# ShannonAI/GNN-LM

Hardware: AMD Instinct MI355X
Metric: eval tokens/sec on WikiText-103 (k=1024, GNN+KNN); test ppl match (higher is better)
Workload: dtype f32

## Files before the change

### gnn-lm_amd/csrc/ivfpq8_scan.hip

```cpp
#include "kernels.h"
#include "ivfpq8_layout.h"

namespace gnnlm {
namespace {

typedef int v4i __attribute__((ext_vector_type(4)));
typedef int v8i __attribute__((ext_vector_type(8)));
typedef unsigned u32x2 __attribute__((ext_vector_type(2)));
typedef unsigned v4u __attribute__((ext_vector_type(4)));

#define GNNLM_PERM(hi_, lo_, sel_) __builtin_amdgcn_perm((hi_), (lo_), (sel_))
#ifndef GNNLM_IVF8_NW
#define GNNLM_IVF8_NW 16
#endif
constexpr int NW = GNNLM_IVF8_NW, NTH = 64 * NW;
#ifndef GNNLM_IVF8_PF
#define GNNLM_IVF8_PF 3
#endif
#ifndef GNNLM_IVF8_PF_SUMS
#define GNNLM_IVF8_PF_SUMS 3
#endif
template <bool SUMS>
__global__ __launch_bounds__(NTH) void ivfpq_scan8_kernel(gnnlm_ivfpq_scan8_t p) {
    extern __shared__ __attribute__((aligned(16))) unsigned char smem[];
// ... 235 lines not shown
        for (int q = 0; q < 4; ++q) lookups4(C[0], q, X[q]);
#define GNNLM_IVF8_STEP(t) if constexpr (PF > (t)) { step(C[((t) + 1) % PF], C[(t)], u); u += NW * TS; }
        while (u < nt) {
            GNNLM_IVF8_STEP(0) GNNLM_IVF8_STEP(1) GNNLM_IVF8_STEP(2) GNNLM_IVF8_STEP(3)
            GNNLM_IVF8_STEP(4) GNNLM_IVF8_STEP(5) GNNLM_IVF8_STEP(6) GNNLM_IVF8_STEP(7)
        }
#undef GNNLM_IVF8_STEP
        static_assert(PF >= 3 && PF <= 8, "GNNLM_IVF8_PF");
    }
    if (SUMS) {
        __syncthreads();
#pragma unroll
        for (int u = 0; u < QG; ++u) {
            const int64_t ob = p.grp_out[(int64_t)grp * QG + u];
            if (qs[u] < 0 || ob < 0) continue;
            for (int e = tid; e < HIST_BINS; e += NTH) p.out_hist[ob + e] = hist[u * HIST_BINS + e];
        }
        advance_slow();
        continue;
    }
    count_entries(wgc);
    if (tid == 0) *next_s = next_index();
    __syncthreads();
    if (tid < QG) {
        const int tot = wgc[tid];
        wgc[tid] = (tot > 0 && qs_lane >= 0) ? atomicAdd(&p.surv_cnt[(int64_t)qs_lane * SURV_CNT_STRIDE], tot) : 0;
    }
    __syncthreads();
    gi_next = *next_s;
    write_entries(wgc);
    }
}

__global__ __launch_bounds__(1024) void ivfpq_tau_kernel(gnnlm_ivfpq_tau_t p) {
    constexpr int CB = 2 * HIST_BINS;
    __shared__ int comb[CB];
    __shared__ int part[1024];
    __shared__ int bstar_s;
    const int tid = threadIdx.x;
    const int64_t q = blockIdx.x;
    const float delta = p.qmeta[q * 4], sum_lo = p.qmeta[q * 4 + 1], amax = p.qmeta[q * 4 + 2];
    float bmin = INFINITY, bmax = -INFINITY;
    for (int d = 0; d < p.D; ++d) {
        if (p.probe_list[q * p.ld_probe + d] < 0) continue;
        const float b = p.probe_bias[q * p.ld_probe + d];
        bmin = fminf(bmin, b);
        bmax = fmaxf(bmax, b);
    }
    int c0 = 0, c1 = 0;
    for (int d = 0; d < p.D; ++d) {
        if (p.probe_list[q * p.ld_probe + d] < 0) continue;
        const float offf = (p.probe_bias[q * p.ld_probe + d] - bmin) / delta * 0.9999f - 1.f;
        const int sh = (int)fminf(fmaxf(offf, 0.f), (float)(HIST_BINS << HIST_SHIFT)) >> HIST_SHIFT;
        const uint32_t* h = p.hist + (q * p.D + d) * HIST_BINS;
        const int b0 = tid - sh, b1 = tid + 1024 - sh;
        if (b0 >= 0 && b0 < HIST_BINS) c0 += (int)h[b0];
        if (b1 >= 0 && b1 < HIST_BINS) c1 += (int)h[b1];
    }
    comb[tid] = c0;
    comb[tid + 1024] = c1;
    if (tid == 0) bstar_s = -1;
    __syncthreads();
    const int h0 = comb[2 * tid], h1 = comb[2 * tid + 1], mine = h0 + h1;
    part[tid] = mine;
    __syncthreads();
    int suf = mine;
    for (int step = 1; step < 1024; step <<= 1) {
        const int other = tid + step < 1024 ? part[tid + step] : 0;
        __syncthreads();
        suf += other;
        part[tid] = suf;
        __syncthreads();
    }
    if (suf >= p.k && suf - mine < p.k) bstar_s = (suf - mine + h1 >= p.k) ? 2 * tid + 1 : 2 * tid;
    __syncthreads();
    if (tid == 0) {
        float tau = -INFINITY;
        if (bstar_s >= 0) {
            const float eps = 66.f * 2.3841858e-7f * (64.f * amax + fmaxf(fabsf(bmin), fabsf(bmax)));
            tau = (bmin + sum_lo) + (float)(bstar_s << HIST_SHIFT) * delta * (1.f - 6.1035156e-5f) - eps;
            tau -= fabsf(tau) * 2.3841858e-7f + 1e-30f;
        }
        p.tau[q] = tau;
    }
}

}

int ivfpq_scan8(const gnnlm_ivfpq_scan8_t& d, hipStream_t stream) {
    GNNLM_REQUIRE(d.max_groups >= 0, "ivfpq_scan8: bad group count");
    if (d.max_groups == 0) return OK;
    GNNLM_REQUIRE(d.tiles && d.list_off && d.qlut && d.qmeta && d.coarse && d.grp_list && d.grp_q && d.n_groups &&
                      (d.out_hist || (d.tau && d.surv && d.surv_cnt && d.cap > 0)),
                  "ivfpq_scan8: null operand");
    GNNLM_REQUIRE(d.M == 64 && (uintptr_t)d.tiles % 16 == 0 && (uintptr_t)d.qlut % 4 == 0, "ivfpq_scan8: need M = 64, aligned images");
    GNNLM_REQUIRE(!d.out_hist || d.grp_out, "ivfpq_scan8: out_hist needs grp_out");
    GNNLM_REQUIRE(d.nlist > 0 && d.nlist <= (1 << SURV_LIST_BITS) && d.max_list >= 0 && d.max_list < (1ll << SURV_ROW_BITS),
                  "ivfpq_scan8: the survivor records hold 18 bits of list and 19 bits of row: need 0 < nlist <= 2^18 and max_list < 2^19");
    GNNLM_LDS_OPT_IN(&ivfpq_scan8_kernel<false>, scan8_lds(false));
    GNNLM_LDS_OPT_IN(&ivfpq_scan8_kernel<true>, scan8_lds(true));
    ProfScope prof(d.out_hist ? K_IVF8S : K_IVF8, stream, 0.0, 0.0);
    int dev = 0, cus = 0;
    GNNLM_HIP(hipGetDevice(&dev));
    GNNLM_HIP(hipDeviceGetAttribute(&cus, hipDeviceAttributeMultiprocessorCount, dev));
    const dim3 grid((unsigned)scan8_grid(d.max_groups, cus));
    if (d.out_hist) hipLaunchKernelGGL(ivfpq_scan8_kernel<true>, grid, dim3(NTH), scan8_lds(true), stream, d);
    else hipLaunchKernelGGL(ivfpq_scan8_kernel<false>, grid, dim3(NTH), scan8_lds(false), stream, d);
    GNNLM_LAUNCH_CHECK();
    return OK;
}

int ivfpq_tau(const gnnlm_ivfpq_tau_t& d, hipStream_t stream) {
    GNNLM_REQUIRE(d.n >= 0 && d.n < (1ll << 31) && d.D >= 1 && d.k > 0, "ivfpq_tau: bad shape");
    if (d.n == 0) return OK;
    GNNLM_REQUIRE(d.hist && d.probe_list && d.probe_bias && d.qmeta && d.tau && d.ld_probe >= d.D, "ivfpq_tau: null operand");
    ProfScope prof(K_TAU, stream, 0.0, 4.0 * (double)d.n * d.D * HIST_BINS);
    hipLaunchKernelGGL(ivfpq_tau_kernel, dim3((unsigned)d.n), dim3(1024), 0, stream, d);
    GNNLM_LAUNCH_CHECK();
    return OK;
}

}
```

### gnn-lm_amd/csrc/ivfpq_select.hip

```cpp
#include <cmath>
#include <cstdint>

#include "kernels.h"

namespace gnnlm {
namespace {

__device__ __forceinline__ uint32_t key_of(float v) {
    const uint32_t u = __float_as_uint(v);
    return (u & 0x80000000u) ? ~u : (u | 0x80000000u);
}
__device__ __forceinline__ float value_of_key(uint32_t key) { return __uint_as_float((key & 0x80000000u) ? (key & 0x7fffffffu) : ~key); }

struct ProbeParams {
    const float* scores; int64_t ld; int64_t n; int ncols;
    const float* col_bias;
    int k, largest;
    float* out_val; int64_t* out_id;
};

__device__ __forceinline__ int wave_count(bool pred) { return __popcll(__ballot(pred)); }

template <int NCH>
__global__ __launch_bounds__(256) void ivfpq_select_probes_kernel(ProbeParams p) {
// ... 87 lines not shown
    for (int r = 0; r < NR; ++r) {
        const int col = 256 * (r / 4) + 4 * lane + (r % 4);
        uint64_t m = __ballot(key[r] > T || (key[r] == T && col <= C));
        while (m) {
            const int src = __builtin_ctzll(m);
            m &= m - 1;
            const uint32_t kv = (uint32_t)__builtin_amdgcn_readlane((int)key[r], src);
            if (lane == base) { okey = kv; ocol = 256 * (r / 4) + 4 * src + (r % 4); }
            ++base;
        }
    }
    unsigned long long s = okey ? ((unsigned long long)okey << 32) | (unsigned)(4095 - ocol) : 0ull;
#pragma unroll
    for (int size = 2; size <= 64; size <<= 1) {
#pragma unroll
        for (int d = size >> 1; d > 0; d >>= 1) {
            const unsigned long long o = __shfl_xor(s, d, 64);
            const bool keep_max = ((lane & d) == 0) == ((lane & size) == 0);
            s = keep_max ? (s > o ? s : o) : (s < o ? s : o);
        }
    }
    if (lane < p.k) {
        const uint32_t kk = (uint32_t)(s >> 32);
        p.out_val[row * p.k + lane] = kk ? sign * value_of_key(kk) : (p.largest ? NEG : INFINITY);
        p.out_id[row * p.k + lane] = kk ? (int64_t)(4095 - (int)(uint32_t)s) : (int64_t)-1;
    }
}

struct FinalParams {
    const float* val; int64_t ld_val; const int64_t* ids; int64_t ld_ids;
    const int32_t* row_ncols; int64_t n; int cap, k;
    float* out_val; int64_t* out_id;
    int label_bits; int32_t val_last; int32_t* out_vals;
};

template <int EPT>
__global__ __launch_bounds__(256) void ivfpq_select_final_kernel(FinalParams p) {
    constexpr int NT = 256, NB = 2048, KP = 1024;
    __shared__ int64_t id[2][KP];
    __shared__ float val[2][KP];
    __shared__ int hist[NB];
    __shared__ int wtot[4];
    __shared__ float wext[4][2];
    __shared__ int dig_s, above_s, cnt;
    const int tid = threadIdx.x, lane = tid & 63, wave = tid >> 6;
    const int64_t row = blockIdx.x;
    const float NEG = -INFINITY;
    const float* srow = p.val + row * p.ld_val;
    const int64_t* irow = p.ids + row * p.ld_ids;
    const int ncols = p.row_ncols ? min(p.cap, p.row_ncols[row]) : p.cap;
    auto entry = [&](int c, float& v, uint32_t& key, int64_t& cid) -> bool {
        v = srow[c] + 0.f;
        cid = irow[c];
        key = key_of(v);
        return cid >= 0 && v > NEG;
    };
    auto pick = [&](int need) -> int {
        int own[8], mine = 0;
#pragma unroll
        for (int b = 0; b < 8; ++b) { own[b] = hist[8 * tid + b]; mine += own[b]; }
        int suf = mine;
#pragma unroll
        for (int d = 1; d < 64; d <<= 1) {
            const int o = __shfl_down(suf, d, 64);
            if (lane + d < 64) suf += o;
        }
        if (lane == 0) wtot[wave] = suf;
        if (tid == 0) { dig_s = -1; above_s = 0; }
        __syncthreads();
        for (int w = wave + 1; w < 4; ++w) suf += wtot[w];
        if (suf >= need && suf - mine < need) {
            int acc_ = suf - mine;
#pragma unroll
            for (int b = 7; b >= 0; --b) {
                if (acc_ + own[b] >= need) { dig_s = 8 * tid + b; above_s = acc_; break; }
                acc_ += own[b];
            }
        }
        __syncthreads();
        return dig_s;
    };
    uint32_t rkey[EPT];
    int64_t rid[EPT];
// ... 151 lines not shown
            if (p.label_bits > 0 && p.out_vals) p.out_vals[o] = (int32_t)(pid & ((1ll << p.label_bits) - 1));
        }
    }
    for (int e = m + tid; e < p.k; e += NT) {
        const int64_t o = row * p.k + e;
        p.out_val[o] = NEG;
        p.out_id[o] = -1;
        if (p.label_bits > 0 && p.out_vals) p.out_vals[o] = p.val_last;
    }
}

}

int ivfpq_select_probes(const gnnlm_ivfpq_select_probes_t& d, hipStream_t stream) {
    GNNLM_REQUIRE(d.out_val && d.out_id && d.k > 0 && d.k <= 64, "ivfpq_select_probes: need output buffers and 0 < k <= 64");
    GNNLM_REQUIRE(d.n >= 0 && d.n < (1ll << 31) && d.ncols >= 0 && d.ncols <= 4096, "ivfpq_select_probes: need 0 <= ncols <= 4096");
    if (d.n == 0) return OK;
    GNNLM_REQUIRE(d.ncols == 0 || d.scores, "ivfpq_select_probes: null scores");
    ProbeParams p{d.scores, d.ld, d.n, d.ncols, d.col_bias, d.k, d.largest, d.out_val, d.out_id};
    ProfScope prof(K_TOPK, stream, 0.0, 4.0 * (double)d.n * d.ncols + 12.0 * (double)d.n * d.k);
    const dim3 grid((unsigned)cdiv(d.n, 4)), block(256);
    if (d.ncols <= 256) hipLaunchKernelGGL(ivfpq_select_probes_kernel<1>, grid, block, 0, stream, p);
    else if (d.ncols <= 1024) hipLaunchKernelGGL(ivfpq_select_probes_kernel<4>, grid, block, 0, stream, p);
    else hipLaunchKernelGGL(ivfpq_select_probes_kernel<16>, grid, block, 0, stream, p);
    GNNLM_LAUNCH_CHECK();
    return OK;
}

int ivfpq_select_final(const gnnlm_ivfpq_select_final_t& d, hipStream_t stream) {
    GNNLM_REQUIRE(d.out_val && d.out_id && d.k > 0 && d.k <= 1024, "ivfpq_select_final: need output buffers and 0 < k <= 1024");
    GNNLM_REQUIRE(d.n >= 0 && d.n < (1ll << 31) && d.cap >= 0 && d.cap <= 16384, "ivfpq_select_final: need 0 <= cap <= 16384");
    GNNLM_REQUIRE(d.label_bits >= 0 && d.label_bits < 32, "ivfpq_select_final: need 0 <= label_bits < 32");
    if (d.n == 0) return OK;
    GNNLM_REQUIRE(d.cap == 0 || (d.cand_val && d.cand_id), "ivfpq_select_final: null candidates");
    FinalParams p{d.cand_val, d.ld_val, d.cand_id, d.ld_id, d.row_ncols, d.n, d.cap, d.k, d.out_val, d.out_id,
                  d.label_bits, d.val_last, d.out_vals};
    ProfScope prof(K_TOPK, stream, 0.0, 12.0 * (double)d.n * d.cap + 16.0 * (double)d.n * d.k);
    const dim3 grid((unsigned)d.n), block(256);
    if (d.cap <= 4096) hipLaunchKernelGGL(ivfpq_select_final_kernel<16>, grid, block, 0, stream, p);
    else hipLaunchKernelGGL(ivfpq_select_final_kernel<20>, grid, block, 0, stream, p);
    GNNLM_LAUNCH_CHECK();
    return OK;
}

}
```

### gnn-lm_amd/ivfpq.py

```python
import contextlib
import ctypes
import os
from collections import namedtuple
from typing import NamedTuple, Optional

import numpy as np
import torch

from . import _lib, ivfpq_train, ops


class _LazyStats(dict):

    def add(self, key, thunk):
        dict.setdefault(self, key, 0)
        self.__dict__.setdefault("_pending", {}).setdefault(key, []).append(thunk)

    def set(self, key, value):
        dict.__setitem__(self, key, value)

    def _resolve(self, key):
        pend = self.__dict__.get("_pending", {}).pop(key, None)
        if pend:
            dict.__setitem__(self, key, dict.__getitem__(self, key) + sum(t() for t in pend))
# ... 389 lines not shown
            _lib.call("gnnlm_ivfpq_pack_lut", _lib.ptr(blk.lut), blk.lut.stride(0), nq, self.M, _lib.ptr(lut_s), _lib.stream())
        ov = torch.empty(nq, dense * self.max_list, device=dev, dtype=torch.float32)
        self._scan(lut_s, blk, 0, dense, out=ov)
        ops.topk_merge(ov, bv, bi, largest=True, init=True)
        lst = torch.gather(pi, 1, torch.div(bi, self.max_list, rounding_mode="floor").clamp_(0, dense - 1))
        pos = self.list_off[lst.clamp(min=0)] + bi % self.max_list
        bi.copy_(torch.where(torch.isinf(bv) | (lst < 0), torch.full_like(bi, -1), self.payload[pos.clamp_(0, max(self.ntotal - 1, 0))]))
        if plan.nprobe <= dense:
            return None
        tau = torch.where(bi[:, k - 1] >= 0, bv[:, k - 1], torch.full_like(bv[:, k - 1], float("-inf"))).contiguous()
        self._scan(lut_s, blk, dense, plan.nprobe, filt=(tau, plan.cap))
        stats.add("candidates", lambda cc=blk.cc: cc.sum().double())
        if self.keep_candidates:
            self.last_candidates = (blk.cv, blk.ci, blk.cc, tau)
        ops.topk_merge(blk.cv, bv, bi, ids=blk.ci, largest=True, init=False, row_ncols=blk.cc.clamp(max=plan.cap))
        return blk.cc

    def _block_int8(self, plan, blk, out, stats):
        dev, nq, pi, cc = self.device, blk.pv.shape[0], blk.pi, blk.cc
        hist = torch.empty(nq, plan.dense, self.HIST_BINS, device=dev, dtype=torch.int32)
        self._scan8(blk.tables, blk.cs, self._groups(pi[:, :plan.dense], seg=self.HIST_BINS), hist=hist, stride=plan.S)
        tau = self._tau(plan, blk, hist)
        surv = torch.empty(nq, plan.cap, 2, device=dev, dtype=torch.int32)
        sc16 = torch.zeros(nq, self.CNT_STRIDE, device=dev, dtype=torch.int32)
        g2 = self._groups(pi)
        stats.add("groups", lambda g=g2[2]: g[0].double())
        self._scan8(blk.tables, blk.cs, g2, filt=(tau, surv, sc16))
        sc = sc16[:, 0]
        self._rescore(plan, blk, (tau, surv, sc16), stats)
        stats.add("survivors", lambda sc=sc: sc.sum().double())
        stats.add("candidates", lambda cc=cc: cc.sum().double())
        if self.keep_candidates:
            self.last_candidates = (blk.cv, blk.ci, cc, tau)
        self._select_final(plan, blk, out)
        over = sc
        if plan.ccap < plan.cap:
            over = torch.where(cc > plan.ccap, torch.full_like(sc, self.COLUMNS), over)
        if plan.S > 1:
            avail = self.list_len[pi.clamp(min=0)].masked_fill(pi < 0, 0).sum(1)
            short = cc.to(torch.int64) < avail.clamp(max=plan.k)
            stats.add("underflow", lambda short=short: short.sum().double())
            over = torch.where(short, torch.full_like(sc, self.UNDERFLOW), over)
        return over

    def _select_probes(self, plan, cs, pv, pi, col_bias=None):
        ops.ivfpq_select_probes(cs, pv, pi, col_bias, plan.select)

    def _tables_begin(self, qr):
        nq, dev = qr.shape[0], self.device
        lut = torch.empty(nq, self.M * 256, device=dev, dtype=torch.float32)
        tables = side = None
        if self.route == "int8":
            tables = (torch.empty(nq, *self.QLUT_SHAPE, dtype=torch.uint8, device=dev), torch.empty(nq, self.QMETA, dtype=torch.float32, device=dev))
            if not torch.cuda.is_current_stream_capturing():
                cur = torch.cuda.current_stream()
                side = self._side_streams.get(cur.cuda_stream)
                if side is None:
                    side = self._side_streams[cur.cuda_stream] = torch.cuda.Stream(device=dev)
                side.wait_stream(cur)
        with torch.cuda.stream(side) if side is not None else contextlib.nullcontext():
            if tables is not None and self.dsub in (4, 8, 16, 32):
                t = _lib.gnnlm_ivfpq_tables_t()
                t.qr, t.ld_qr, t.n, t.pq, t.M, t.dsub = qr.data_ptr(), qr.stride(0), nq, self.pq.data_ptr(), self.M, self.dsub
                t.lut, t.ld_lut, t.qlut, t.qmeta = lut.data_ptr(), lut.stride(0), tables[0].data_ptr(), tables[1].data_ptr()
                _lib.call_desc("gnnlm_ivfpq_tables", t)
                return lut, tables, side
            g = _lib.gnnlm_gemm_t()
# ... 48 lines not shown
        d.qlut, d.qmeta, d.coarse, d.ld_coarse = tables[0].data_ptr(), tables[1].data_ptr(), cs.data_ptr(), cs.stride(0)
        d.grp_list, d.grp_q, d.n_groups, d.max_groups = groups[0].data_ptr(), groups[1].data_ptr(), groups[2].data_ptr(), groups[3]
        ctr = torch.zeros(*self.WORK_CTR_SHAPE, device=self.device, dtype=torch.int32)
        d.work_ctr = ctr.data_ptr()
        if hist is not None:
            d.out_hist, d.grp_out = hist.data_ptr(), groups[4].data_ptr()
        else:
            tau, surv, cnt = filt
            d.tau, d.surv, d.surv_cnt, d.cap = tau.data_ptr(), surv.data_ptr(), cnt.data_ptr(), surv.shape[1]
        _lib.call_desc("gnnlm_ivfpq_scan8", d)

    def _tau(self, plan, blk, hist):
        tau = torch.empty(hist.shape[0], device=self.device, dtype=torch.float32)
        t = _lib.gnnlm_ivfpq_tau_t()
        t.hist, t.D = hist.data_ptr(), plan.dense
        t.probe_list, t.probe_bias, t.ld_probe = blk.pi.data_ptr(), blk.pv.data_ptr(), blk.pi.stride(0)
        t.qmeta, t.n, t.k, t.tau = blk.tables[1].data_ptr(), hist.shape[0], plan.rank, tau.data_ptr()
        _lib.call_desc("gnnlm_ivfpq_tau", t)
        return tau

    def _rescore(self, plan, blk, filt, stats):
        tau, surv, sc16 = filt
        r = _lib.gnnlm_ivfpq_rescore_t()
        r.codes, r.payload, r.M = self.list_codes.data_ptr(), self.payload.data_ptr(), self.M
        r.lut, r.ld_lut, r.coarse, r.ld_coarse, r.tau = blk.lut.data_ptr(), blk.lut.stride(0), blk.cs.data_ptr(), blk.cs.stride(0), tau.data_ptr()
        r.surv, r.surv_cnt, r.cap, r.n = surv.data_ptr(), sc16.data_ptr(), plan.cap, sc16.shape[0]
        r.cand_val, r.cand_id, r.cand_cnt, r.cand_cap = blk.cv.data_ptr(), blk.ci.data_ptr(), blk.cc.data_ptr(), plan.ccap
        if self.refine_tau:
            rc16 = torch.empty_like(sc16)
            r.qmeta, r.k, r.out_cnt = blk.tables[1].data_ptr(), plan.k, rc16.data_ptr()
            stats.add("rescored", lambda rc=rc16: rc[:, 0].sum().double())
        _lib.call_desc("gnnlm_ivfpq_rescore", r)

    def _select_final(self, plan, blk, out):
        cv, ci, ccap = blk.cv, blk.ci, plan.ccap
        if not (plan.k <= 1024 and (out.split or plan.select)):
            return ops.topk_merge(cv, out.val, out.idx, ids=ci, largest=True, init=True, row_ncols=blk.cc.clamp(max=ccap))
        rn = blk.cc.clamp(max=ccap)
        f = _lib.gnnlm_ivfpq_select_final_t()
        f.cand_val, f.ld_val, f.cand_id, f.ld_id = cv.data_ptr(), cv.stride(0), ci.data_ptr(), ci.stride(0)
        f.row_ncols, f.n, f.cap, f.k, f.out_val, f.out_id = rn.data_ptr(), cv.shape[0], ccap, plan.k, out.val.data_ptr(), out.idx.data_ptr()
        if out.split:
            f.label_bits, f.val_last = self.LABEL_BITS, self.val_last
            if out.labels is not None:
                f.out_vals = out.labels.data_ptr()
        _lib.call_desc("gnnlm_ivfpq_select_final", f)
```

### include/gnnlm.h

```cpp
#ifndef GNNLM_H
#define GNNLM_H

#include <stddef.h>
#include <stdint.h>

#ifdef __cplusplus
extern "C" {
#endif

#define GNNLM_ABI_VERSION 12
#define GNNLM_OK 0
#define GNNLM_E_INVALID (-22)
#define GNNLM_E_NOMEM (-12)
#define GNNLM_E_HIP (-5)

const char* gnnlm_last_error(void);
int gnnlm_abi_version(void);
const char* gnnlm_target_arch(void);
size_t gnnlm_sizeof(const char* struct_name);

typedef struct gnnlm_gemm {
    const float* A;  int64_t lda;
    const int32_t* a_rows;
    const float* W;  int64_t ldw;
// ... 279 lines not shown
    const int32_t* n_groups;  int32_t max_groups;
    uint32_t* surv;  int32_t* surv_cnt;  int32_t cap;
    uint32_t* out_hist;  const int64_t* grp_out;
    int32_t sums_stride;
    int32_t* work_ctr;
    int32_t nlist;  int64_t max_list;
} gnnlm_ivfpq_scan8_t;
int gnnlm_ivfpq_scan8(const gnnlm_ivfpq_scan8_t* desc, void* stream);
typedef struct gnnlm_ivfpq_tau {
    const uint32_t* hist;  int32_t D;
    const int64_t* probe_list;  const float* probe_bias;  int32_t ld_probe;
    const float* qmeta;
    int64_t n;  int32_t k;
    float* tau;
} gnnlm_ivfpq_tau_t;
int gnnlm_ivfpq_tau(const gnnlm_ivfpq_tau_t* desc, void* stream);
int gnnlm_ivfpq_split_payload(int64_t* idx, int64_t n, int32_t label_bits, int32_t val_last, int32_t* out_vals, void* stream);
typedef struct gnnlm_ivfpq_select_probes {
    const float* scores;  int64_t ld;
    int64_t n;  int32_t ncols;
    const float* col_bias;
    int32_t k;
    int32_t largest;
    float* out_val;  int64_t* out_id;
} gnnlm_ivfpq_select_probes_t;
int gnnlm_ivfpq_select_probes(const gnnlm_ivfpq_select_probes_t* desc, void* stream);
typedef struct gnnlm_ivfpq_select_final {
    const float* cand_val;  int64_t ld_val;
    const int64_t* cand_id;  int64_t ld_id;
    const int32_t* row_ncols;
    int64_t n;  int32_t cap;  int32_t k;
    float* out_val;  int64_t* out_id;
    int32_t label_bits;  int32_t val_last;  int32_t* out_vals;
} gnnlm_ivfpq_select_final_t;
int gnnlm_ivfpq_select_final(const gnnlm_ivfpq_select_final_t* desc, void* stream);
typedef struct gnnlm_ivfpq_rescore {
    const uint8_t* codes;  const int64_t* payload;
    int32_t M;
    const float* lut;  int64_t ld_lut;
    const float* coarse;  int64_t ld_coarse;
    const float* tau;
    const uint32_t* surv;  const int32_t* surv_cnt;  int32_t cap;
    int64_t n;
    float* cand_val;  int64_t* cand_id;  int32_t* cand_cnt;  int32_t cand_cap;
    const float* qmeta;  int32_t k;  int32_t* out_cnt;
} gnnlm_ivfpq_rescore_t;
int gnnlm_ivfpq_rescore(const gnnlm_ivfpq_rescore_t* desc, void* stream);
typedef struct gnnlm_ivfpq_encode {
    const float* x;  int64_t ldx;  int64_t n;
    const int64_t* assign;
    const float* coarse;  int32_t nlist;
    const float* pq;  const float* norm2;
    int32_t M;  int32_t dsub;  int32_t d;
    uint8_t* codes;  int64_t ld_codes;
    int64_t* list_cnt;  int32_t* n_bad;
} gnnlm_ivfpq_encode_t;
int gnnlm_ivfpq_encode_rows(const gnnlm_ivfpq_encode_t* desc, void* stream);
typedef struct gnnlm_ivfpq_list_merge {
    const int64_t* list_off_old;  int32_t nlist;  int64_t N0;
    const int64_t* ids_old;  const uint8_t* codes_old;  int32_t M;
    int64_t n;  const int64_t* dest;  const int64_t* ids_new;  const uint8_t* codes_new;  int64_t ld_new;
    const int64_t* new_off;
    int64_t* ids;  uint8_t* codes;
    int32_t* n_bad;
} gnnlm_ivfpq_list_merge_t;
int gnnlm_ivfpq_list_merge(const gnnlm_ivfpq_list_merge_t* desc, void* stream);
typedef struct gnnlm_ivfpq_coarse {
// ... 302 lines not shown
```

### gnn-lm_amd/csrc/ivfpq8_layout.h

```cpp
#pragma once
#include <stddef.h>
#include <stdint.h>

#if defined(__HIPCC__)
#include <hip/hip_runtime.h>
#define GNNLM_HD __host__ __device__
#else
#define GNNLM_HD
#endif

namespace gnnlm {

constexpr int QG = 8;
constexpr int TQ = 32;
constexpr int QLUT_BYTES = 64 * 256;
constexpr int TAB_BYTES = 2 * 256 * 32 * QG;
#ifndef GNNLM_IVF8_WAVE_CAP
#define GNNLM_IVF8_WAVE_CAP 240
#endif
constexpr int WAVE_CAP = GNNLM_IVF8_WAVE_CAP;
constexpr int SCAN_CTL = 768;
constexpr int SCAN_LDS = TAB_BYTES + SCAN_CTL + 16 * WAVE_CAP * 8;
constexpr int HIST_BINS = 1024, HIST_SHIFT = 4;
constexpr int SUMS_LDS = TAB_BYTES + QG * HIST_BINS * 4;
constexpr int SURV_CNT_STRIDE = 16;
static_assert(TAB_BYTES == QG * QLUT_BYTES, "a group's LDS tables are its queries' byte tables, interleaved");
static_assert(SCAN_LDS <= 160 * 1024 && SUMS_LDS <= 160 * 1024, "the scan's tables + staging regions / histograms exceed a CU's LDS");

constexpr int SURV_ROW_BITS = 19, SURV_LIST_BITS = 18, SURV_EXCESS_MAX = 254, SURV_SUM_BIG = 16383;
static_assert(SURV_SUM_BIG == (1 << (32 - SURV_LIST_BITS)) - 1 && SURV_SUM_BIG > 16320, "list and sum share the record's second word");
struct SurvRec { uint32_t row, word; };
GNNLM_HD constexpr SurvRec surv_pack(uint32_t row, uint32_t list, uint32_t sum) { return SurvRec{row, list | sum << SURV_LIST_BITS}; }
GNNLM_HD constexpr uint32_t surv_list(uint32_t word) { return word & ((1u << SURV_LIST_BITS) - 1u); }
GNNLM_HD constexpr uint32_t surv_sum(uint32_t word) { return word >> SURV_LIST_BITS; }

constexpr int64_t ivf8_cdiv(int64_t a, int64_t b) { return (a + b - 1) / b; }
constexpr int64_t groups_cap(int64_t n, int64_t P, int64_t nlist) { return n * P / QG + nlist + 1; }
constexpr int64_t groups_fill(int64_t G, int64_t nlist) { return G * QG > 2 * (nlist + 1) ? G * QG : 2 * (nlist + 1); }
constexpr int64_t scan8_grid(int64_t max_groups, int64_t cus) {
    const int64_t by_groups = 8 * ivf8_cdiv(max_groups, 8), by_cus = 8 * ivf8_cdiv(cus > 8 ? cus : 8, 8);
    return by_groups < by_cus ? by_groups : by_cus;
}
constexpr size_t scan8_lds(bool sums) { return sums ? SUMS_LDS : SCAN_LDS; }
constexpr size_t rescore_lds(int M, int threads) { return (size_t)M * 256 * 4 + (size_t)threads * M; }
constexpr int64_t tables_grid(int64_t n) { return ivf8_cdiv(n, TQ); }

#if defined(__HIPCC__)
__device__ __forceinline__ int filter_threshold(const float* __restrict__ qmeta, int64_t q, float bias, float tau) {
    const float delta = qmeta[q * 4], sum_lo = qmeta[q * 4 + 1], amax = qmeta[q * 4 + 2];
    const float eps = 66.f * 2.3841858e-7f * (64.f * amax + fabsf(bias) + (fabsf(tau) < INFINITY ? fabsf(tau) : 0.f));
    const float thr = ((tau - bias) - sum_lo - eps) / delta - 64.f;
    return !(thr == thr) || thr <= -1.0e9f ? -(1 << 30) : (thr >= 1.0e9f ? 0x7fffffff : (int)floorf(thr) - 128 * 64);
}
#endif

}
```

### gnn-lm_amd/csrc/ivfpq8_rescore.hip

```cpp
#include "kernels.h"
#include "ivfpq8_layout.h"

namespace gnnlm {
namespace {

typedef unsigned v4u __attribute__((ext_vector_type(4)));
#ifndef GNNLM_REFINE_NT
#define GNNLM_REFINE_NT 1024
#endif
template <int EPT>
__device__ __forceinline__ void refine_wg(const gnnlm_ivfpq_rescore_t& p, const int64_t q, int* hist, int& n_left, float& tau_left) {
    constexpr int NT = GNNLM_REFINE_NT, NB = 2048, NWV = NT / 64;
    __shared__ int wtot[NWV];
    __shared__ int dig_s, base_s;
    const int tid = threadIdx.x, lane = tid & 63, wave = tid >> 6;
    const int n = min(p.surv_cnt[q * SURV_CNT_STRIDE], p.cap);
    uint2* surv = reinterpret_cast<uint2*>(const_cast<uint32_t*>(p.surv)) + q * p.cap;
    const float tau0 = p.tau[q];
    n_left = n;
    tau_left = tau0;
    if (n < p.k || !(tau0 > -INFINITY)) {
        if (tid == 0 && p.out_cnt) p.out_cnt[q * SURV_CNT_STRIDE] = n;
        return;
    }
// ... 109 lines not shown
            uint2 rec = uint2{0u, 0u};
            bool keep = false;
            if (c < n) { rec = surv[c]; keep = keep_rec(rec); }
            const uint64_t m = __builtin_amdgcn_ballot_w64(keep);
            const int rank = __builtin_amdgcn_mbcnt_hi((uint32_t)(m >> 32), __builtin_amdgcn_mbcnt_lo((uint32_t)m, 0u));
            __syncthreads();
            if (lane == 0) wtot[wave] = __builtin_popcountll(m);
            __syncthreads();
            int before = base_s;
            for (int w = 0; w < wave; ++w) before += wtot[w];
            if (keep) surv[before + rank] = rec;
            __syncthreads();
            if (tid == 0) { int tot = 0; for (int w = 0; w < NWV; ++w) tot += wtot[w]; base_s += tot; }
            __syncthreads();
        }
        total = base_s;
    }
    if (tid == 0) {
        if (p.out_cnt) p.out_cnt[q * SURV_CNT_STRIDE] = total;
        const_cast<float*>(p.tau)[q] = tau1;
    }
    n_left = total;
    tau_left = tau1;
}

#ifndef GNNLM_RESCORE_NT
#define GNNLM_RESCORE_NT 1024
#endif
template <int M, bool TAB_READY>
__device__ __forceinline__ void rescore_wg(const gnnlm_ivfpq_rescore_t& p, const int64_t q, const int n, const float tau, float* rtab) {
    __shared__ int ccnt;
    constexpr int NT = GNNLM_RESCORE_NT;
    uint32_t* cdw = reinterpret_cast<uint32_t*>(rtab + M * 256);
    const int tid = threadIdx.x;
    if (tid == 0) ccnt = 0;
    const uint2* surv = reinterpret_cast<const uint2*>(p.surv) + q * p.cap;
    const int last = max(n - 1, 0);
    auto record = [&](int e, uint2& rec) __attribute__((always_inline)) { rec = surv[min(e, last)]; };
    auto rowload = [&](const uint2& rec, v4u (&cr)[M / 16], float& bias) __attribute__((always_inline)) {
        bias = p.coarse[q * p.ld_coarse + surv_list(rec.y)];
        const v4u* crow = reinterpret_cast<const v4u*>(p.codes + (int64_t)rec.x * M);
#pragma unroll
        for (int c16 = 0; c16 < M / 16; ++c16) cr[c16] = crow[c16];
    };
    uint2 recC = uint2{0u, 0u}, recD = recC;
    v4u cr0[M / 16], cr1[M / 16];
    float bias0 = 0.f, bias1 = 0.f;
    uint32_t rid0 = 0u, rid1 = 0u;
    if (n > 0) {
        if (!TAB_READY) {
            const float4* src = reinterpret_cast<const float4*>(p.lut + q * p.ld_lut);
            float4* dst = reinterpret_cast<float4*>(rtab);
            for (int e = tid; e < M * 64; e += NT) dst[e] = src[e];
        }
        uint2 r0, r1;
        record(tid, r0);
        record(tid + NT, r1);
        record(tid + 2 * NT, recC);
        rowload(r0, cr0, bias0);
        rid0 = r0.x;
        rowload(r1, cr1, bias1);
        rid1 = r1.x;
    }
    __syncthreads();
    const uint8_t* cb = reinterpret_cast<const uint8_t*>(cdw + tid);
    auto one = [&](int e, v4u (&cr)[M / 16], float& bset, uint32_t& rset, const uint2& rec_old, uint2& rec_new) __attribute__((always_inline)) {
        const int64_t row = rset;
        const float bias = bset;
#pragma unroll
        for (int c16 = 0; c16 < M / 16; ++c16) {
            cdw[(4 * c16 + 0) * NT + tid] = cr[c16].x;
            cdw[(4 * c16 + 1) * NT + tid] = cr[c16].y;
            cdw[(4 * c16 + 2) * NT + tid] = cr[c16].z;
            cdw[(4 * c16 + 3) * NT + tid] = cr[c16].w;
        }
        record(e + 3 * NT, rec_new);
        rowload(rec_old, cr, bset);
        rset = rec_old.x;
        const int rot = (int)(row & 31);
        float a0 = 0.f, a1 = 0.f;
#pragma unroll
        for (int h = 0; h < M / 32; ++h) {
#pragma unroll 8
            for (int s = 0; s < 32; s += 2) {
                const int m0 = 32 * h + ((rot + s) & 31), m1 = 32 * h + ((rot + s + 1) & 31);
                a0 = a0 + rtab[m0 * 256 + cb[(m0 >> 2) * (4 * NT) + (m0 & 3)]];
                a1 = a1 + rtab[m1 * 256 + cb[(m1 >> 2) * (4 * NT) + (m1 & 3)]];
            }
        }
        const float score = bias + (a0 + a1);
        if (score > tau) {
            const int pos = atomicAdd(&ccnt, 1);
            if (pos < p.cand_cap) {
                p.cand_val[q * p.cand_cap + pos] = score;
                p.cand_id[q * p.cand_cap + pos] = row;
            }
        }
    };
    int e = tid;
#pragma unroll
    for (int it = 0; it < 8; ++it) {
        if (e >= n) break;
        one(e, cr0, bias0, rid0, recC, recD);
        e += NT;
        if (e >= n) break;
        one(e, cr1, bias1, rid1, recD, recC);
        e += NT;
    }
    for (; e < n; e += 2 * NT) {
        one(e, cr0, bias0, rid0, recC, recD);
        if (e + NT >= n) break;
        one(e + NT, cr1, bias1, rid1, recD, recC);
    }
    __syncthreads();
    if (tid == 0) p.cand_cnt[q] = ccnt;
    const int nc = min(ccnt, p.cand_cap);
    for (int e = tid; e < nc; e += NT) p.cand_id[q * p.cand_cap + e] = p.payload[p.cand_id[q * p.cand_cap + e]];
}

template <int M>
__global__ __launch_bounds__(GNNLM_RESCORE_NT) void ivfpq_rescore_kernel(gnnlm_ivfpq_rescore_t p) {
    extern __shared__ __attribute__((aligned(16))) float rtab[];
    const int64_t q = blockIdx.x;
    rescore_wg<M, false>(p, q, min(p.surv_cnt[q * SURV_CNT_STRIDE], p.cap), p.tau[q], rtab);
}

static_assert(GNNLM_REFINE_NT == GNNLM_RESCORE_NT, "the fused refine + re-score launch runs both on one workgroup shape");
template <int EPT>
__global__ __launch_bounds__(GNNLM_RESCORE_NT) void ivfpq_refine_rescore_kernel(gnnlm_ivfpq_rescore_t p) {
    constexpr int M = 64;
    extern __shared__ __attribute__((aligned(16))) float rtab[];
    const int tid = threadIdx.x, lane = tid & 63, wave = tid >> 6;
    const int64_t q = blockIdx.x;
    const int n0 = min(p.surv_cnt[q * SURV_CNT_STRIDE], p.cap);
    if (n0 > 0) {
        const float* src = p.lut + q * p.ld_lut + (4 * wave) * 256 + 4 * lane;
        const unsigned dst = (unsigned)(uintptr_t)(__attribute__((address_space(3))) void*)rtab + (unsigned)(4 * __builtin_amdgcn_readfirstlane(wave)) * 1024u;
        unsigned keep_;
        asm volatile("s_mov_b32 %0, m0\n\ts_mov_b32 m0, %2\n\ts_nop 0\n\t"
                     "global_load_lds_dwordx4 %1, off\n\tglobal_load_lds_dwordx4 %1, off offset:1024\n\t"
                     "global_load_lds_dwordx4 %1, off offset:2048\n\tglobal_load_lds_dwordx4 %1, off offset:3072\n\t"
                     "s_mov_b32 m0, %0"
                     : "=&s"(keep_) : "v"(src), "s"(dst) : "memory");
    }
    int n_left;
    float tau_left;
    refine_wg<EPT>(p, q, reinterpret_cast<int*>(rtab + M * 256), n_left, tau_left);
    asm volatile("s_waitcnt vmcnt(0)" ::: "memory");
    __syncthreads();
    rescore_wg<M, true>(p, q, n_left, tau_left, rtab);
}

__global__ __launch_bounds__(256) void split_payload_kernel(int64_t* __restrict__ idx, int64_t n, int label_bits, int32_t val_last, int32_t* __restrict__ out_vals) {
    const int64_t e = (int64_t)blockIdx.x * 256 + threadIdx.x;
    if (e >= n) return;
    const int64_t v = idx[e];
    idx[e] = v < 0 ? v : v >> label_bits;
    if (out_vals) out_vals[e] = v < 0 ? val_last : (int32_t)(v & ((1ll << label_bits) - 1));
}

}

int ivfpq_rescore(const gnnlm_ivfpq_rescore_t& d, hipStream_t stream) {
    GNNLM_REQUIRE(d.n >= 0 && d.n < (1ll << 31), "ivfpq_rescore: bad query count");
    if (d.n == 0) return OK;
    GNNLM_REQUIRE(d.codes && d.payload && d.lut && d.coarse && d.tau && d.surv && d.surv_cnt && d.cand_val && d.cand_id && d.cand_cnt &&
                      d.cap > 0 && d.cand_cap > 0,
                  "ivfpq_rescore: null operand");
    GNNLM_REQUIRE(d.M == 64 && d.ld_lut >= (int64_t)d.M * 256 && d.ld_lut % 4 == 0 && (uintptr_t)d.lut % 16 == 0 &&
                      (uintptr_t)d.codes % 16 == 0,
                  "ivfpq_rescore: need M = 64, 16-byte aligned tables");
    ProfScope prof(K_RESCORE, stream, 0.0, 0.0);
    const size_t lds = rescore_lds(d.M, GNNLM_RESCORE_NT);
    if (d.qmeta) {
        GNNLM_REQUIRE(d.k > 0, "ivfpq_rescore: the refinement needs k > 0");
        GNNLM_LDS_OPT_IN(&ivfpq_refine_rescore_kernel<8>, lds);
        hipLaunchKernelGGL(ivfpq_refine_rescore_kernel<8>, dim3((unsigned)d.n), dim3(GNNLM_RESCORE_NT), lds, stream, d);
    } else {
        GNNLM_LDS_OPT_IN(&ivfpq_rescore_kernel<64>, lds);
        hipLaunchKernelGGL(ivfpq_rescore_kernel<64>, dim3((unsigned)d.n), dim3(GNNLM_RESCORE_NT), lds, stream, d);
    }
    GNNLM_LAUNCH_CHECK();
    return OK;
}

int ivfpq_split_payload(int64_t* idx, int64_t n, int label_bits, int32_t val_last, int32_t* out_vals, hipStream_t stream) {
    GNNLM_REQUIRE(idx && n >= 0 && label_bits > 0 && label_bits < 32, "ivfpq_split_payload: bad arguments");
    if (n == 0) return OK;
    hipLaunchKernelGGL(split_payload_kernel, dim3((unsigned)cdiv(n, (int64_t)256)), dim3(256), 0, stream, idx, n, label_bits, val_last, out_vals);
    GNNLM_LAUNCH_CHECK();
    return OK;
}

}
```

Before: 572,100.

## Compute IVF tau per wave and fuse overflow flags into final select

Adds a tau kernel that assigns one wavefront per query instead of a 1024-thread block. Each lane accumulates a window of shifted histogram bins in registers using 16-byte loads, and a DPP suffix sum replaces the LDS scan and its barriers. The final select kernel now also computes each row's overflow/underflow status (survivor count, column cap, sampled-list availability), replacing several separate torch elementwise ops on the host path. This adds register pressure and more code paths; both changes are gated by environment variables.

Measured after the change: 576,400, median of 6. Within noise of the previous version (+0.8%).

```diff
diff --git a/gnn-lm_amd/csrc/ivfpq8_scan.hip b/gnn-lm_amd/csrc/ivfpq8_scan.hip
--- a/gnn-lm_amd/csrc/ivfpq8_scan.hip
+++ b/gnn-lm_amd/csrc/ivfpq8_scan.hip
@@ -291,6 +291,83 @@
     }
 }
 
+constexpr int TAU_W = 2 * HIST_BINS / 64;
+static_assert(TAU_W % 4 == 0 && TAU_W * 64 == 2 * HIST_BINS, "a lane's window of combined bins is whole 16-byte pieces");
+template <int R>
+__device__ __forceinline__ void tau_add_window(int (&c)[TAU_W], const uint4 (&w)[TAU_W / 4 + 1]) {
+#pragma unroll
+    for (int j = 0; j < TAU_W; ++j) {
+        const int i = j + 4 - R;
+        const uint4 v = w[i >> 2];
+        c[j] += (int)((i & 3) == 0 ? v.x : (i & 3) == 1 ? v.y : (i & 3) == 2 ? v.z : v.w);
+    }
+}
+__device__ __forceinline__ int wave_suffix_sum(int v) {
+    v += __builtin_amdgcn_update_dpp(0, v, 0x101, 0xf, 0xf, true);
+    v += __builtin_amdgcn_update_dpp(0, v, 0x102, 0xf, 0xf, true);
+    v += __builtin_amdgcn_update_dpp(0, v, 0x104, 0xf, 0xf, true);
+    v += __builtin_amdgcn_update_dpp(0, v, 0x108, 0xf, 0xf, true);
+    const int t1 = __builtin_amdgcn_readlane(v, 16), t2 = __builtin_amdgcn_readlane(v, 32), t3 = __builtin_amdgcn_readlane(v, 48);
+    const int row = (threadIdx.x & 63) >> 4;
+    return v + (row == 0 ? t1 + t2 + t3 : row == 1 ? t2 + t3 : row == 2 ? t3 : 0);
+}
+__device__ __forceinline__ float tau_of_bin(int bstar, float bmin, float bmax, float delta, float sum_lo, float amax) {
+    const float eps = 66.f * 2.3841858e-7f * (64.f * amax + fmaxf(fabsf(bmin), fabsf(bmax)));
+    float tau = (bmin + sum_lo) + (float)(bstar << HIST_SHIFT) * delta * (1.f - 6.1035156e-5f) - eps;
+    tau -= fabsf(tau) * 2.3841858e-7f + 1e-30f;
+    return tau;
+}
+__global__ __launch_bounds__(256) void ivfpq_tau_wave_kernel(gnnlm_ivfpq_tau_t p) {
+    const int lane = threadIdx.x & 63;
+    const int64_t q = (int64_t)blockIdx.x * 4 + (threadIdx.x >> 6);
+    if (q >= p.n) return;
+    const float delta = p.qmeta[q * 4], sum_lo = p.qmeta[q * 4 + 1], amax = p.qmeta[q * 4 + 2];
+    float bmin = INFINITY, bmax = -INFINITY;
+    for (int d = 0; d < p.D; ++d) {
+        if (p.probe_list[q * p.ld_probe + d] < 0) continue;
+        const float b = p.probe_bias[q * p.ld_probe + d];
+        bmin = fminf(bmin, b);
+        bmax = fmaxf(bmax, b);
+    }
+    int c[TAU_W];
+#pragma unroll
+    for (int j = 0; j < TAU_W; ++j) c[j] = 0;
+    for (int d = 0; d < p.D; ++d) {
+        if (p.probe_list[q * p.ld_probe + d] < 0) continue;
+        const float offf = (p.probe_bias[q * p.ld_probe + d] - bmin) / delta * 0.9999f - 1.f;
+        const int sh = (int)fminf(fmaxf(offf, 0.f), (float)(HIST_BINS << HIST_SHIFT)) >> HIST_SHIFT;
+        const uint4* h4 = reinterpret_cast<const uint4*>(p.hist + (q * p.D + d) * HIST_BINS);
+        const int g0 = lane * (TAU_W / 4) - (sh >> 2) - 1;
+        uint4 w[TAU_W / 4 + 1];
+#pragma unroll
+        for (int i = 0; i <= TAU_W / 4; ++i) {
+            const int g = g0 + i;
+            w[i] = g >= 0 && g < HIST_BINS / 4 ? h4[g] : make_uint4(0u, 0u, 0u, 0u);
+        }
+        switch (sh & 3) {
+            case 0: tau_add_window<0>(c, w); break;
+            case 1: tau_add_window<1>(c, w); break;
+            case 2: tau_add_window<2>(c, w); break;
+            default: tau_add_window<3>(c, w); break;
+        }
+    }
+    int mine = 0;
+#pragma unroll
+    for (int j = 0; j < TAU_W; ++j) mine += c[j];
+    const int suf = wave_suffix_sum(mine);
+    if (suf >= p.k && suf - mine < p.k) {
+        int acc = suf - mine, bstar = -1;
+#pragma unroll
+        for (int j = TAU_W - 1; j >= 0; --j) {
+            acc += c[j];
+            if (bstar < 0 && acc >= p.k) bstar = lane * TAU_W + j;
+        }
+        p.tau[q] = tau_of_bin(bstar, bmin, bmax, delta, sum_lo, amax);
+    } else if (lane == 0 && suf < p.k) {
+        p.tau[q] = -INFINITY;
+    }
+}
+
 __global__ __launch_bounds__(1024) void ivfpq_tau_kernel(gnnlm_ivfpq_tau_t p) {
     constexpr int CB = 2 * HIST_BINS;
     __shared__ int comb[CB];
@@ -334,13 +411,7 @@
     if (suf >= p.k && suf - mine < p.k) bstar_s = (suf - mine + h1 >= p.k) ? 2 * tid + 1 : 2 * tid;
     __syncthreads();
     if (tid == 0) {
-        float tau = -INFINITY;
-        if (bstar_s >= 0) {
-            const float eps = 66.f * 2.3841858e-7f * (64.f * amax + fmaxf(fabsf(bmin), fabsf(bmax)));
-            tau = (bmin + sum_lo) + (float)(bstar_s << HIST_SHIFT) * delta * (1.f - 6.1035156e-5f) - eps;
-            tau -= fabsf(tau) * 2.3841858e-7f + 1e-30f;
-        }
-        p.tau[q] = tau;
+        p.tau[q] = bstar_s >= 0 ? tau_of_bin(bstar_s, bmin, bmax, delta, sum_lo, amax) : -INFINITY;
     }
 }
 
@@ -374,7 +445,11 @@
     if (d.n == 0) return OK;
     GNNLM_REQUIRE(d.hist && d.probe_list && d.probe_bias && d.qmeta && d.tau && d.ld_probe >= d.D, "ivfpq_tau: null operand");
     ProfScope prof(K_TAU, stream, 0.0, 4.0 * (double)d.n * d.D * HIST_BINS);
-    hipLaunchKernelGGL(ivfpq_tau_kernel, dim3((unsigned)d.n), dim3(1024), 0, stream, d);
+    static const bool per_wave = [] { const char* e = getenv("GNNLM_IVF_TAU"); return !(e && e[0] == '0' && !e[1]); }();
+    if (per_wave && (uintptr_t)d.hist % 16 == 0)
+        hipLaunchKernelGGL(ivfpq_tau_wave_kernel, dim3((unsigned)cdiv(d.n, 4)), dim3(256), 0, stream, d);
+    else
+        hipLaunchKernelGGL(ivfpq_tau_kernel, dim3((unsigned)d.n), dim3(1024), 0, stream, d);
     GNNLM_LAUNCH_CHECK();
     return OK;
 }
diff --git a/gnn-lm_amd/csrc/ivfpq_select.hip b/gnn-lm_amd/csrc/ivfpq_select.hip
--- a/gnn-lm_amd/csrc/ivfpq_select.hip
+++ b/gnn-lm_amd/csrc/ivfpq_select.hip
@@ -143,6 +143,8 @@
     const int32_t* row_ncols; int64_t n; int cap, k;
     float* out_val; int64_t* out_id;
     int label_bits; int32_t val_last; int32_t* out_vals;
+    const int32_t* surv_cnt; int64_t ld_surv_cnt; const int64_t* probe_list; int64_t ld_probe; int nprobe;
+    const int64_t* list_len; int surv_cap, sampled; int32_t* out_over;
 };
 
 template <int EPT>
@@ -160,6 +162,22 @@
     const float* srow = p.val + row * p.ld_val;
     const int64_t* irow = p.ids + row * p.ld_ids;
     const int ncols = p.row_ncols ? min(p.cap, p.row_ncols[row]) : p.cap;
+    if (p.out_over && wave == 0) {
+        const int c = p.row_ncols[row];
+        int over = p.surv_cnt[row * p.ld_surv_cnt];
+        if (p.cap < p.surv_cap && c > p.cap) over = GNNLM_IVFPQ_OVER_COLUMNS;
+        if (p.sampled) {
+            int avail = 0;
+            for (int j = lane; j < p.nprobe; j += 64) {
+                const int64_t l = p.probe_list[row * p.ld_probe + j];
+                if (l >= 0) avail = (int)min((int64_t)avail + p.list_len[l], (int64_t)p.k);
+            }
+#pragma unroll
+            for (int d = 1; d < 64; d <<= 1) avail += __shfl_xor(avail, d, 64);
+            if (c < min(avail, p.k)) over = GNNLM_IVFPQ_OVER_UNDERFLOW;
+        }
+        if (lane == 0) p.out_over[row] = over;
+    }
     auto entry = [&](int c, float& v, uint32_t& key, int64_t& cid) -> bool {
         v = srow[c] + 0.f;
         cid = irow[c];
@@ -377,9 +395,12 @@
     GNNLM_REQUIRE(d.n >= 0 && d.n < (1ll << 31) && d.cap >= 0 && d.cap <= 16384, "ivfpq_select_final: need 0 <= cap <= 16384");
     GNNLM_REQUIRE(d.label_bits >= 0 && d.label_bits < 32, "ivfpq_select_final: need 0 <= label_bits < 32");
     if (d.n == 0) return OK;
+    GNNLM_REQUIRE(!d.out_over || (d.row_ncols && d.surv_cnt && (!d.sampled || (d.nprobe >= 0 && (d.nprobe == 0 || (d.probe_list && d.list_len))))),
+                  "ivfpq_select_final: out_over needs row_ncols, surv_cnt and, sampled, the probes with the lists' lengths");
     GNNLM_REQUIRE(d.cap == 0 || (d.cand_val && d.cand_id), "ivfpq_select_final: null candidates");
     FinalParams p{d.cand_val, d.ld_val, d.cand_id, d.ld_id, d.row_ncols, d.n, d.cap, d.k, d.out_val, d.out_id,
-                  d.label_bits, d.val_last, d.out_vals};
+                  d.label_bits, d.val_last, d.out_vals,
+                  d.surv_cnt, d.ld_surv_cnt, d.probe_list, d.ld_probe, d.nprobe, d.list_len, d.surv_cap, d.sampled, d.out_over};
     ProfScope prof(K_TOPK, stream, 0.0, 12.0 * (double)d.n * d.cap + 16.0 * (double)d.n * d.k);
     const dim3 grid((unsigned)d.n), block(256);
     if (d.cap <= 4096) hipLaunchKernelGGL(ivfpq_select_final_kernel<16>, grid, block, 0, stream, p);
diff --git a/gnn-lm_amd/ivfpq.py b/gnn-lm_amd/ivfpq.py
--- a/gnn-lm_amd/ivfpq.py
+++ b/gnn-lm_amd/ivfpq.py
@@ -445,7 +445,11 @@
         stats.add("candidates", lambda cc=cc: cc.sum().double())
         if self.keep_candidates:
             self.last_candidates = (blk.cv, blk.ci, cc, tau)
-        self._select_final(plan, blk, out)
+        over = self._select_final(plan, blk, out, sc16)
+        if over is not None:
+            if plan.S > 1:
+                stats.add("underflow", lambda o=over: (o >= self.UNDERFLOW).sum().double())
+            return over
         over = sc
         if plan.ccap < plan.cap:
             over = torch.where(cc > plan.ccap, torch.full_like(sc, self.COLUMNS), over)
@@ -560,11 +564,13 @@
             stats.add("rescored", lambda rc=rc16: rc[:, 0].sum().double())
         _lib.call_desc("gnnlm_ivfpq_rescore", r)
 
-    def _select_final(self, plan, blk, out):
+    def _select_final(self, plan, blk, out, sc16=None):
         cv, ci, ccap = blk.cv, blk.ci, plan.ccap
         if not (plan.k <= 1024 and (out.split or plan.select)):
-            return ops.topk_merge(cv, out.val, out.idx, ids=ci, largest=True, init=True, row_ncols=blk.cc.clamp(max=ccap))
-        rn = blk.cc.clamp(max=ccap)
+            ops.topk_merge(cv, out.val, out.idx, ids=ci, largest=True, init=True, row_ncols=blk.cc.clamp(max=ccap))
+            return None
+        fused = sc16 is not None and os.environ.get("GNNLM_IVF_OVER", "1") != "0"
+        rn = blk.cc if fused else blk.cc.clamp(max=ccap)
         f = _lib.gnnlm_ivfpq_select_final_t()
         f.cand_val, f.ld_val, f.cand_id, f.ld_id = cv.data_ptr(), cv.stride(0), ci.data_ptr(), ci.stride(0)
         f.row_ncols, f.n, f.cap, f.k, f.out_val, f.out_id = rn.data_ptr(), cv.shape[0], ccap, plan.k, out.val.data_ptr(), out.idx.data_ptr()
@@ -572,4 +578,10 @@
             f.label_bits, f.val_last = self.LABEL_BITS, self.val_last
             if out.labels is not None:
                 f.out_vals = out.labels.data_ptr()
+        over = None
+        if fused:
+            over = torch.empty(cv.shape[0], device=cv.device, dtype=torch.int32)
+            f.surv_cnt, f.ld_surv_cnt, f.surv_cap, f.sampled, f.out_over = sc16.data_ptr(), sc16.stride(0), plan.cap, int(plan.S > 1), over.data_ptr()
+            f.probe_list, f.ld_probe, f.nprobe, f.list_len = blk.pi.data_ptr(), blk.pi.stride(0), blk.pi.shape[1], self.list_len.data_ptr()
         _lib.call_desc("gnnlm_ivfpq_select_final", f)
+        return over
diff --git a/include/gnnlm.h b/include/gnnlm.h
--- a/include/gnnlm.h
+++ b/include/gnnlm.h
@@ -335,7 +335,14 @@
     int64_t n;  int32_t cap;  int32_t k;
     float* out_val;  int64_t* out_id;
     int32_t label_bits;  int32_t val_last;  int32_t* out_vals;
+    const int32_t* surv_cnt;  int64_t ld_surv_cnt;
+    const int64_t* probe_list;  int64_t ld_probe;  int32_t nprobe;
+    const int64_t* list_len;
+    int32_t surv_cap;  int32_t sampled;
+    int32_t* out_over;
 } gnnlm_ivfpq_select_final_t;
+#define GNNLM_IVFPQ_OVER_UNDERFLOW (1 << 30)
+#define GNNLM_IVFPQ_OVER_COLUMNS ((1 << 30) - 1)
 int gnnlm_ivfpq_select_final(const gnnlm_ivfpq_select_final_t* desc, void* stream);
 typedef struct gnnlm_ivfpq_rescore {
     const uint8_t* codes;  const int64_t* payload;
```

## Stage rescore candidates in LDS and rewrite tau kernel with wave-level scans

Applied to the files above, without the earlier changes.

The rescore kernel now writes the first few thousand above-threshold candidates (score, row) into an LDS staging area instead of global memory. It then does the payload gather and the final global writes in a batched pass, so the global read-after-write of cand_id goes away for staged entries. The tau kernel loads probe metadata eight probes per lane and broadcasts it with readlane, batches the histogram loads, and replaces the block-wide LDS suffix scan with wave shuffles plus a 16-entry wave-total array. This cuts barriers and serial per-probe loads, at the cost of more LDS per rescore workgroup and more register use.

Measured after the change: 570,900 before, 574,700 after, median of 6. No clear change (+0.7%).

```diff
diff --git a/gnn-lm_amd/csrc/ivfpq8_layout.h b/gnn-lm_amd/csrc/ivfpq8_layout.h
--- a/gnn-lm_amd/csrc/ivfpq8_layout.h
+++ b/gnn-lm_amd/csrc/ivfpq8_layout.h
@@ -43,6 +43,9 @@
 }
 constexpr size_t scan8_lds(bool sums) { return sums ? SUMS_LDS : SCAN_LDS; }
 constexpr size_t rescore_lds(int M, int threads) { return (size_t)M * 256 * 4 + (size_t)threads * M; }
+constexpr int RESCORE_STAGE_SLOTS = 2560;
+constexpr size_t RESCORE_STAGE_BYTES = (size_t)RESCORE_STAGE_SLOTS * 8;
+static_assert(rescore_lds(64, 1024) + RESCORE_STAGE_BYTES + 1024 <= 160 * 1024, "the re-score's table + code rows + candidate staging exceed a CU's LDS");
 constexpr int64_t tables_grid(int64_t n) { return ivf8_cdiv(n, TQ); }
 
 #if defined(__HIPCC__)
diff --git a/gnn-lm_amd/csrc/ivfpq8_rescore.hip b/gnn-lm_amd/csrc/ivfpq8_rescore.hip
--- a/gnn-lm_amd/csrc/ivfpq8_rescore.hip
+++ b/gnn-lm_amd/csrc/ivfpq8_rescore.hip
@@ -165,6 +165,9 @@
     __shared__ int ccnt;
     constexpr int NT = GNNLM_RESCORE_NT;
     uint32_t* cdw = reinterpret_cast<uint32_t*>(rtab + M * 256);
+    float* sval = reinterpret_cast<float*>(cdw + (M / 4) * NT);
+    uint32_t* srow = reinterpret_cast<uint32_t*>(sval + RESCORE_STAGE_SLOTS);
+    const int s_eff = min(RESCORE_STAGE_SLOTS, p.cand_cap);
     const int tid = threadIdx.x;
     if (tid == 0) ccnt = 0;
     const uint2* surv = reinterpret_cast<const uint2*>(p.surv) + q * p.cap;
@@ -224,7 +227,10 @@
         const float score = bias + (a0 + a1);
         if (score > tau) {
             const int pos = atomicAdd(&ccnt, 1);
-            if (pos < p.cand_cap) {
+            if (pos < s_eff) {
+                sval[pos] = score;
+                srow[pos] = (uint32_t)row;
+            } else if (pos < p.cand_cap) {
                 p.cand_val[q * p.cand_cap + pos] = score;
                 p.cand_id[q * p.cand_cap + pos] = row;
             }
@@ -248,7 +254,25 @@
     __syncthreads();
     if (tid == 0) p.cand_cnt[q] = ccnt;
     const int nc = min(ccnt, p.cand_cap);
-    for (int e = tid; e < nc; e += NT) p.cand_id[q * p.cand_cap + e] = p.payload[p.cand_id[q * p.cand_cap + e]];
+    constexpr int SPT = (RESCORE_STAGE_SLOTS + NT - 1) / NT;
+    const int ns = min(nc, s_eff);
+    int64_t pay[SPT];
+#pragma unroll
+    for (int j = 0; j < SPT; ++j) {
+        const int e = tid + j * NT;
+        pay[j] = e < ns ? p.payload[srow[e]] : 0;
+    }
+#pragma unroll
+    for (int j = 0; j < SPT; ++j) {
+        const int e = tid + j * NT;
+        if (e < ns) p.cand_val[q * p.cand_cap + e] = sval[e];
+    }
+#pragma unroll
+    for (int j = 0; j < SPT; ++j) {
+        const int e = tid + j * NT;
+        if (e < ns) p.cand_id[q * p.cand_cap + e] = pay[j];
+    }
+    for (int e = s_eff + tid; e < nc; e += NT) p.cand_id[q * p.cand_cap + e] = p.payload[p.cand_id[q * p.cand_cap + e]];
 }
 
 template <int M>
@@ -304,7 +328,7 @@
                       (uintptr_t)d.codes % 16 == 0,
                   "ivfpq_rescore: need M = 64, 16-byte aligned tables");
     ProfScope prof(K_RESCORE, stream, 0.0, 0.0);
-    const size_t lds = rescore_lds(d.M, GNNLM_RESCORE_NT);
+    const size_t lds = rescore_lds(d.M, GNNLM_RESCORE_NT) + RESCORE_STAGE_BYTES;
     if (d.qmeta) {
         GNNLM_REQUIRE(d.k > 0, "ivfpq_rescore: the refinement needs k > 0");
         GNNLM_LDS_OPT_IN(&ivfpq_refine_rescore_kernel<8>, lds);
diff --git a/gnn-lm_amd/csrc/ivfpq8_scan.hip b/gnn-lm_amd/csrc/ivfpq8_scan.hip
--- a/gnn-lm_amd/csrc/ivfpq8_scan.hip
+++ b/gnn-lm_amd/csrc/ivfpq8_scan.hip
@@ -294,53 +294,72 @@
 __global__ __launch_bounds__(1024) void ivfpq_tau_kernel(gnnlm_ivfpq_tau_t p) {
     constexpr int CB = 2 * HIST_BINS;
     __shared__ int comb[CB];
-    __shared__ int part[1024];
-    __shared__ int bstar_s;
-    const int tid = threadIdx.x;
+    __shared__ int wtot[16];
+    const int tid = threadIdx.x, lane = tid & 63, wave = tid >> 6;
     const int64_t q = blockIdx.x;
     const float delta = p.qmeta[q * 4], sum_lo = p.qmeta[q * 4 + 1], amax = p.qmeta[q * 4 + 2];
+    constexpr int DU = 8;
+    const int du = lane & (DU - 1);
+    const int64_t* plist = p.probe_list + q * p.ld_probe;
+    const float* pbias = p.probe_bias + q * p.ld_probe;
+    auto probe = [&](int d0, float& b) -> bool {
+        const int d = min(d0 + du, p.D - 1);
+        b = pbias[d];
+        return (plist[d] >= 0) & (d0 + du < p.D);
+    };
+    auto lane_f = [](float x, int l) -> float { return __int_as_float(__builtin_amdgcn_readlane(__float_as_int(x), l)); };
     float bmin = INFINITY, bmax = -INFINITY;
-    for (int d = 0; d < p.D; ++d) {
-        if (p.probe_list[q * p.ld_probe + d] < 0) continue;
-        const float b = p.probe_bias[q * p.ld_probe + d];
-        bmin = fminf(bmin, b);
-        bmax = fmaxf(bmax, b);
+    for (int d0 = 0; d0 < p.D; d0 += DU) {
+        float b;
+        const bool on = probe(d0, b);
+        const float lo = on ? b : INFINITY, hi = on ? b : -INFINITY;
+#pragma unroll
+        for (int u = 0; u < DU; ++u) {
+            bmin = fminf(bmin, lane_f(lo, u));
+            bmax = fmaxf(bmax, lane_f(hi, u));
+        }
     }
     int c0 = 0, c1 = 0;
-    for (int d = 0; d < p.D; ++d) {
-        if (p.probe_list[q * p.ld_probe + d] < 0) continue;
-        const float offf = (p.probe_bias[q * p.ld_probe + d] - bmin) / delta * 0.9999f - 1.f;
-        const int sh = (int)fminf(fmaxf(offf, 0.f), (float)(HIST_BINS << HIST_SHIFT)) >> HIST_SHIFT;
-        const uint32_t* h = p.hist + (q * p.D + d) * HIST_BINS;
-        const int b0 = tid - sh, b1 = tid + 1024 - sh;
-        if (b0 >= 0 && b0 < HIST_BINS) c0 += (int)h[b0];
-        if (b1 >= 0 && b1 < HIST_BINS) c1 += (int)h[b1];
+    for (int d0 = 0; d0 < p.D; d0 += DU) {
+        float b;
+        const bool on = probe(d0, b);
+        const float offf = (b - bmin) / delta * 0.9999f - 1.f;
+        const int sh_l = on ? (int)fminf(fmaxf(offf, 0.f), (float)(HIST_BINS << HIST_SHIFT)) >> HIST_SHIFT : -1;
+        int sh[DU];
+        uint32_t hv[DU];
+#pragma unroll
+        for (int u = 0; u < DU; ++u) {
+            sh[u] = __builtin_amdgcn_readlane(sh_l, u);
+            const int d = min(d0 + u, p.D - 1);
+            hv[u] = p.hist[(q * p.D + d) * HIST_BINS + ((tid - max(sh[u], 0)) & (HIST_BINS - 1))];
+        }
+#pragma unroll
+        for (int u = 0; u < DU; ++u) {
+            c0 += (uint32_t)sh[u] <= (uint32_t)tid ? (int)hv[u] : 0;
+            c1 += sh[u] > tid ? (int)hv[u] : 0;
+        }
     }
     comb[tid] = c0;
     comb[tid + 1024] = c1;
-    if (tid == 0) bstar_s = -1;
     __syncthreads();
     const int h0 = comb[2 * tid], h1 = comb[2 * tid + 1], mine = h0 + h1;
-    part[tid] = mine;
+    int suf = mine;
+#pragma unroll
+    for (int s = 1; s < 64; s <<= 1) {
+        const int o = __shfl_down(suf, s, 64);
+        if (lane + s < 64) suf += o;
+    }
+    if (lane == 0) wtot[wave] = suf;
     __syncthreads();
-    int suf = mine;
-    for (int step = 1; step < 1024; step <<= 1) {
-        const int other = tid + step < 1024 ? part[tid + step] : 0;
-        __syncthreads();
-        suf += other;
-        part[tid] = suf;
-        __syncthreads();
-    }
-    if (suf >= p.k && suf - mine < p.k) bstar_s = (suf - mine + h1 >= p.k) ? 2 * tid + 1 : 2 * tid;
-    __syncthreads();
-    if (tid == 0) {
-        float tau = -INFINITY;
-        if (bstar_s >= 0) {
-            const float eps = 66.f * 2.3841858e-7f * (64.f * amax + fmaxf(fabsf(bmin), fabsf(bmax)));
-            tau = (bmin + sum_lo) + (float)(bstar_s << HIST_SHIFT) * delta * (1.f - 6.1035156e-5f) - eps;
-            tau -= fabsf(tau) * 2.3841858e-7f + 1e-30f;
-        }
+    for (int w = wave + 1; w < 16; ++w) suf += wtot[w];
+    if (suf >= p.k && suf - mine < p.k) {
+        const int bstar = (suf - mine + h1 >= p.k) ? 2 * tid + 1 : 2 * tid;
+        const float eps = 66.f * 2.3841858e-7f * (64.f * amax + fmaxf(fabsf(bmin), fabsf(bmax)));
+        float tau = (bmin + sum_lo) + (float)(bstar << HIST_SHIFT) * delta * (1.f - 6.1035156e-5f) - eps;
+        tau -= fabsf(tau) * 2.3841858e-7f + 1e-30f;
         p.tau[q] = tau;
+    } else if (tid == 0 && suf < p.k) {
+        p.tau[q] = -INFINITY;
     }
 }
 
```
